# pc2/StencilStream

Hardware: NVIDIA B200
Metric: GCell-updates/s (higher is better)
Workload: dtype f32

## Files before the change

stencilstream_b200/include/StencilStream/cuda/internal/TileKernel.hpp:

```cpp
#pragma once
#include "../../Stencil.hpp"
#include "Helpers.hpp"

#include <cuda_runtime.h>

#include <cstddef>
#include <cstdint>
#include <type_traits>

namespace stencil {
namespace cuda {
namespace internal {

inline constexpr int store_tile = 0, store_grid = 1, store_runtime = 2;

template <typename Cell, int CW> constexpr bool lane_major_tiles() {
#if defined(STST_NO_LANE_MAJOR)
    return false;
#else
    using L = CellLayout<Cell>;
    if (!(CW == 4 || CW == 8))
        return false;
    const unsigned constant = constant_fields_mask<Cell>();
    unsigned evolving = 0;
    for (std::size_t i = 0; i < L::n_planes; i++) {
        if (L::plane_bytes(i) != 4)
            return false;
        if (!((constant >> i) & 1u))
            evolving++;
    }
  #if defined(STST_MIXED_LANE_MAJOR)
    return evolving == 1;
  #else
    return L::n_planes == 1 && evolving == 1;
  #endif
#endif
}

template <typename Cell, std::size_t I> constexpr bool plane_is_lane_major() {
    return ((constant_fields_mask<Cell>() >> I) & 1u) == 0;
}

inline constexpr int window_shift = 0, window_rotate = 1, window_reload = 2;

inline constexpr unsigned max_fused_iterations = 16;

inline constexpr unsigned max_spec_subiterations = 4;

struct SweepGeometry {
    unsigned grid_h, grid_w;
    int buf_row0;
    unsigned buf_rows;
    int out_row_lo;
    int out_row_hi;
    int out2_row_lo;
    int out2_row_hi;
    unsigned tiles_first;
    unsigned tile_h, tile_w;
    unsigned halo;
    unsigned hpad;
    unsigned n_gens;
    unsigned tiles_x;
    unsigned use_tma;
    unsigned push;
    unsigned inv_block_y;
    unsigned keep[max_spec_subiterations];
    unsigned probe;
    unsigned *spec_flags;
    unsigned long long iteration0;
};

template <typename TDV> struct TdvArray {
    TDV v[max_fused_iterations];
};

struct alignas(64) TensorMapSet {
    unsigned char map[max_planes][128];
};

struct HaloPush {
    PlaneSet up, down;
    int up_buf_row0, down_buf_row0;
    int up_row_hi;
    int down_row_lo;
    unsigned *ticket;
    unsigned *flag_up;
    unsigned *flag_down;
    unsigned flag_value;
};


template <typename T, int N> struct alignas((sizeof(T) * N) % 16 == 0 ? 16
                                            : (sizeof(T) * N) % 8 == 0 ? 8
                                            : (sizeof(T) * N) % 4 == 0 ? 4
                                                                       : alignof(T)) Pack {
    T v[N];
};

template <typename T>
inline constexpr bool is_shuffleable_v = std::is_trivially_copyable_v<T> &&
                                         (sizeof(T) == 1 || sizeof(T) == 2 || sizeof(T) == 4 ||
                                          sizeof(T) == 8);


inline constexpr unsigned tile_guard_bytes = 128;

template <typename Cell>
STST_HD inline std::size_t tile_buffer_bytes(unsigned tile_rows, unsigned tile_cols,
                                             unsigned without_planes = 0) {
    using L = CellLayout<Cell>;
    std::size_t total = 0;
    for (std::size_t i = 0; i < L::n_planes; i++) {
        if ((without_planes >> i) & 1u)
            continue;
        std::size_t b = std::size_t(tile_rows) * tile_cols * L::plane_bytes(i);
        total += (b + 127) / 128 * 128;
    }
    return total;
}

template <typename Cell>
STST_HD inline std::size_t tile_smem_bytes(unsigned tile_rows, unsigned tile_cols,
                                           unsigned n_buffers, unsigned single_planes = 0) {
    return tile_buffer_bytes<Cell>(tile_rows, tile_cols) +
           tile_buffer_bytes<Cell>(tile_rows, tile_cols, single_planes) * (n_buffers - 1) +
           2 * tile_guard_bytes;
}

#if defined(__CUDACC__)

template <typename To, typename From> __device__ __forceinline__ To bit_cast_dev(From const &f) {
    static_assert(sizeof(To) >= sizeof(From));
    To t{};
    memcpy(&t, &f, sizeof(From));
    return t;
}

template <typename T> __device__ __forceinline__ T from_bits(unsigned long long bits) {
    T t;
    memcpy(&t, &bits, sizeof(T));
    return t;
}

template <typename T> __device__ __forceinline__ T shuffle_from_lower_lane(T const &v) {
    if constexpr (sizeof(T) <= 4) {
        unsigned bits = bit_cast_dev<unsigned>(v);
        bits = __shfl_up_sync(0xffffffffu, bits, 1);
        return from_bits<T>(bits);
    } else {
        unsigned long long bits = bit_cast_dev<unsigned long long>(v);
        bits = __shfl_up_sync(0xffffffffu, bits, 1);
        return from_bits<T>(bits);
    }
}

template <typename T> __device__ __forceinline__ T shuffle_from_upper_lane(T const &v) {
    if constexpr (sizeof(T) <= 4) {
        unsigned bits = bit_cast_dev<unsigned>(v);
        bits = __shfl_down_sync(0xffffffffu, bits, 1);
        return from_bits<T>(bits);
    } else {
        unsigned long long bits = bit_cast_dev<unsigned long long>(v);
        bits = __shfl_down_sync(0xffffffffu, bits, 1);
        return from_bits<T>(bits);
    }
}

template <int Bytes>
__device__ __forceinline__ void cp_async_group(void *smem_dst, const void *gmem_src) {
    unsigned saddr = static_cast<unsigned>(__cvta_generic_to_shared(smem_dst));
    if constexpr (Bytes % 16 == 0) {
#pragma unroll
        for (int o = 0; o < Bytes; o += 16) {
            asm volatile("cp.async.cg.shared.global [%0], [%1], 16;\n" ::"r"(saddr + o),
                         "l"(static_cast<const char *>(gmem_src) + o)
                         : "memory");
        }
    } else if constexpr (Bytes == 8) {
        asm volatile("cp.async.ca.shared.global [%0], [%1], 8;\n" ::"r"(saddr), "l"(gmem_src)
                     : "memory");
    } else {
        static_assert(Bytes == 4);
        asm volatile("cp.async.ca.shared.global [%0], [%1], 4;\n" ::"r"(saddr), "l"(gmem_src)
                     : "memory");
    }
}

__device__ __forceinline__ void cp_async_wait_all() {
    asm volatile("cp.async.wait_all;\n" ::: "memory");
}


__device__ __forceinline__ void mbarrier_init(unsigned long long *bar, unsigned count) {
    unsigned addr = static_cast<unsigned>(__cvta_generic_to_shared(bar));
    asm volatile("mbarrier.init.shared::cta.b64 [%0], %1;\n" ::"r"(addr), "r"(count) : "memory");
}

__device__ __forceinline__ void fence_mbarrier_init() {
    asm volatile("fence.mbarrier_init.release.cluster;\n" ::: "memory");
}

__device__ __forceinline__ void fence_proxy_async() {
    asm volatile("fence.proxy.async.shared::cta;\n" ::: "memory");
}

__device__ __forceinline__ void mbarrier_arrive_expect_tx(unsigned long long *bar, unsigned bytes) {
    unsigned addr = static_cast<unsigned>(__cvta_generic_to_shared(bar));
    asm volatile("mbarrier.arrive.expect_tx.shared::cta.b64 _, [%0], %1;\n" ::"r"(addr), "r"(bytes)
                 : "memory");
}

__device__ __forceinline__ void mbarrier_wait_parity(unsigned long long *bar, unsigned parity) {
    unsigned addr = static_cast<unsigned>(__cvta_generic_to_shared(bar));
    unsigned done = 0;
    do {
        asm volatile("{\n"
                     ".reg .pred p;\n"
                     "mbarrier.try_wait.parity.shared::cta.b64 p, [%1], %2;\n"
                     "selp.u32 %0, 1, 0, p;\n"
                     "}\n"
                     : "=r"(done)
                     : "r"(addr), "r"(parity)
                     : "memory");
    } while (!done);
}

__device__ __forceinline__ void tma_load_2d(void *smem_dst, const void *tensor_map, int x, int y,
                                            unsigned long long *bar) {
    unsigned dst = static_cast<unsigned>(__cvta_generic_to_shared(smem_dst));
    unsigned mbar = static_cast<unsigned>(__cvta_generic_to_shared(bar));
    asm volatile("cp.async.bulk.tensor.2d.shared::cluster.global.mbarrier::complete_tx::bytes"
                 " [%0], [%1, {%3, %4}], [%2];\n" ::"r"(dst),
                 "l"(tensor_map), "r"(mbar), "r"(x), "r"(y)
                 : "memory");
}


template <typename Cell> struct TileView {
    using L = CellLayout<Cell>;
    unsigned char *base;
    unsigned rows, cols;
    unsigned plane_off[L::n_planes];

    __device__ __forceinline__ TileView(unsigned char *base, unsigned rows, unsigned cols)
        : base(base), rows(rows), cols(cols) {
        unsigned off = 0;
#pragma unroll
        for (unsigned i = 0; i < L::n_planes; i++) {
            plane_off[i] = off;
            unsigned b = rows * cols * unsigned(L::plane_bytes(i));
            off += (b + 127u) / 128u * 128u;
        }
    }

    __device__ __forceinline__ TileView(unsigned char *base, unsigned rows, unsigned cols, int)
        : base(base), rows(rows), cols(cols) {}

    template <std::size_t I> __device__ __forceinline__ typename L::template plane_t<I> *plane() const {
        return reinterpret_cast<typename L::template plane_t<I> *>(base + plane_off[I]);
    }
};


template <typename Cell, int CW, bool kInterior>
__device__ __forceinline__ void stage_tile(TileView<Cell> const &tile, PlaneSet const &src,
                                           TensorMapSet const &maps, SweepGeometry const &geo,
                                           Cell const &halo_value, int gy0, int gx0,
                                           unsigned long long *mbar) {
    using L = CellLayout<Cell>;
    const int c0 = int(threadIdx.x) * CW;
    const int gx = gx0 + c0;

    if (geo.use_tma) {
        if (threadIdx.x == 0 && threadIdx.y == 0) {
            unsigned total = 0;
            for_each_plane<Cell>([&](auto I) {
                total += tile.rows * tile.cols * unsigned(sizeof(typename L::template plane_t<I>));
            });
            mbarrier_arrive_expect_tx(mbar, total);
            for_each_plane<Cell>([&](auto I) {
                tma_load_2d(tile.template plane<I>(), &maps.map[I][0], gx0, gy0 - geo.buf_row0,
                            mbar);
            });
        }
        mbarrier_wait_parity(mbar, 0);
        if constexpr (!kInterior) {
            for (int row = int(threadIdx.y); row < int(tile.rows); row += int(blockDim.y)) {
                const int gy = gy0 + row;
                const bool row_in = gy >= 0 && gy < int(geo.grid_h);
                for_each_plane<Cell>([&](auto I) {
                    auto *s = tile.template plane<I>() + std::size_t(row) * tile.cols + c0;
#pragma unroll
                    for (int i = 0; i < CW; i++) {
                        const bool in = row_in && (gx + i) >= 0 && (gx + i) < int(geo.grid_w);
                        if (!in)
                            s[i] = L::template get<I>(halo_value);
                    }
                });
            }
            __syncthreads();
        }
        return;
    }

    for_each_plane<Cell>([&](auto I) {
        using T = typename L::template plane_t<I>;
        T *sp = tile.template plane<I>();
        const T *gp = static_cast<const T *>(src.base[I]);
        const unsigned long long pitch = src.pitch[I];
        for (int row = int(threadIdx.y); row < int(tile.rows); row += int(blockDim.y)) {
            const int gy = gy0 + row;
            T *s = sp + std::size_t(row) * tile.cols + c0;
            const T *g = gp + (long long)(gy - geo.buf_row0) * (long long)pitch + gx;
            if constexpr (kInterior) {
                if constexpr ((sizeof(T) * CW) % 16 == 0 || sizeof(T) * CW == 8 ||
                              sizeof(T) * CW == 4) {
                    cp_async_group<int(sizeof(T)) * CW>(s, g);
                } else {
                    *reinterpret_cast<Pack<T, CW> *>(s) = *reinterpret_cast<const Pack<T, CW> *>(g);
                }
            } else {
                const bool row_in = gy >= 0 && gy < int(geo.grid_h) &&
                                    unsigned(gy - geo.buf_row0) < geo.buf_rows;
                if (row_in && gx >= 0 && gx + CW <= int(geo.grid_w)) {
                    *reinterpret_cast<Pack<T, CW> *>(s) = *reinterpret_cast<const Pack<T, CW> *>(g);
                } else {
#pragma unroll
                    for (int i = 0; i < CW; i++) {
                        const bool in = row_in && (gx + i) >= 0 && (gx + i) < int(geo.grid_w);
                        s[i] = in ? g[i] : L::template get<I>(halo_value);
                    }
                }
            }
        }
    });
    if constexpr (kInterior)
        cp_async_wait_all();
    __syncthreads();
}


struct SpecTrack {
    unsigned keep;
    unsigned probe;
    unsigned changed;
    unsigned violated;
};

template <typename T> __device__ __forceinline__ bool bits_differ(T const &a, T const &b) {
    if constexpr (sizeof(T) == 1 || sizeof(T) == 2 || sizeof(T) == 4) {
        return bit_cast_dev<unsigned>(a) != bit_cast_dev<unsigned>(b);
    } else if constexpr (sizeof(T) == 8) {
        return bit_cast_dev<unsigned long long>(a) != bit_cast_dev<unsigned long long>(b);
    } else {
        const unsigned char *pa = reinterpret_cast<const unsigned char *>(&a);
        const unsigned char *pb = reinterpret_cast<const unsigned char *>(&b);
        bool d = false;
#pragma unroll
        for (unsigned i = 0; i < sizeof(T); i++)
            d |= pa[i] != pb[i];
        return d;
    }
}

template <typename F, int CW, bool kInterior, int kMode, int kStore, bool kInLaneMajor,
          bool kOutLaneMajor, int kTX, bool kSpec, std::size_t SUB>
__device__ __forceinline__ void
sweep_rows(F const &tf, typename F::Cell const &halo_value,
           typename F::TimeDependentValue const &tdv, std::size_t iteration,
           TileView<typename F::Cell> const &in, TileView<typename F::Cell> const &out,
           bool to_global_arg, PlaneSet const &dst, HaloPush const &push, SweepGeometry const &geo,
           int gy0, int gx0, int row_lo, int row_hi, int out_lo, int out_hi, SpecTrack &spec) {
    using Cell = typename F::Cell;
    using TDV = typename F::TimeDependentValue;
    using L = CellLayout<Cell>;
    using StencilImpl = Stencil<Cell, F::stencil_radius, TDV>;
    constexpr int R = int(F::stencil_radius);
    constexpr int D = 2 * R + 1;
    constexpr int WC = CW + 2 * R;
    static_assert(std::size_t(R) * L::max_plane_bytes() <= tile_guard_bytes,
                  "stencil radius times the widest field exceeds the shared-memory guard");

    const int cols = int(in.cols);
    const int c0 = int(threadIdx.x) * CW;
    const int lane = int(threadIdx.x) & 31;
    const int tx = int(threadIdx.x), TX = kTX ? kTX : int(blockDim.x);
    const bool to_global = kStore == store_runtime ? to_global_arg : (kStore == store_grid);

    const unsigned n_rows = unsigned(row_hi - row_lo);
    const int y_begin =
        row_lo + int((std::uint64_t(n_rows * threadIdx.y) * geo.inv_block_y) >> 24);
    const int y_end =
        row_lo + int((std::uint64_t(n_rows * (threadIdx.y + 1u)) * geo.inv_block_y) >> 24);
    if (y_begin >= y_end)
        return;

#if defined(STST_RELOAD_ROWS)
    constexpr int RPS = (kMode == window_reload) ? STST_RELOAD_ROWS : 1;
#else
    constexpr int RPS = 1;
#endif
    constexpr int DW = D + RPS - 1;
    Cell win[DW][WC];

    auto load_row = [&](Cell(&w)[WC], int row) {
        for_each_plane<Cell>([&](auto I) {
            using T = typename L::template plane_t<I>;
            const T *rp = in.template plane<I>() + row * cols;
            if constexpr (kInLaneMajor && plane_is_lane_major<Cell, I>()) {
                const T *q = rp + tx;
#pragma unroll
                for (int i = 0; i < CW; i++)
                    L::template get<I>(w[R + i]) = q[i * TX];
#pragma unroll
                for (int j = 1; j <= R; j++) {
                    L::template get<I>(w[R - j]) =
                        q[((CW - j % CW) % CW) * TX - (j + CW - 1) / CW];
                    L::template get<I>(w[R + CW - 1 + j]) = q[((j - 1) % CW) * TX + (j - 1) / CW + 1];
                }
                return;
            }
            const Pack<T, CW> p = *reinterpret_cast<const Pack<T, CW> *>(rp + c0);
#pragma unroll
            for (int i = 0; i < CW; i++)
                L::template get<I>(w[R + i]) = p.v[i];
#pragma unroll
            for (int j = 1; j <= R; j++) {
                T left, right;
#if defined(STST_EDGE_SHUFFLES)
                constexpr bool use_shuffles = true;
#else
                constexpr bool use_shuffles = false;
#endif
                if constexpr (is_shuffleable_v<T> && kMode != window_reload && use_shuffles) {
                    static_assert(R <= CW || sizeof(T) == 0,
                                  "edge shuffles reach one lane to each side only");
                    left = shuffle_from_lower_lane(p.v[CW - j]);
                    right = shuffle_from_upper_lane(p.v[j - 1]);
                    if (lane == 0)
                        left = rp[c0 - j];
                    if (lane == 31)
                        right = rp[c0 + CW - 1 + j];
                } else {
                    left = rp[c0 - j];
                    right = rp[c0 + CW - 1 + j];
                }
                L::template get<I>(w[R - j]) = left;
                L::template get<I>(w[R + CW - 1 + j]) = right;
            }
        });
    };

    auto compute_row = [&](auto top_c, int y) {
        constexpr int top = decltype(top_c)::value;
        const int gy = gy0 + y;
        Cell result[CW];
#pragma unroll
        for (int i = 0; i < CW; i++) {
            const int gx = gx0 + c0 + i;
            bool in_grid = true;
            if constexpr (!kInterior) {
                in_grid = gy >= 0 && gy < int(geo.grid_h) && gx >= 0 && gx < int(geo.grid_w);
            }
            if (in_grid) {
                const std::size_t id_r = std::size_t(unsigned(gy)), id_c = std::size_t(unsigned(gx));
                const std::size_t range_r = geo.grid_h, range_c = geo.grid_w;
                if constexpr (kInterior) {
                    __builtin_assume(id_r != 0);
                    __builtin_assume(id_r != range_r - 1);
                    __builtin_assume(id_r < range_r - 1);
                    __builtin_assume(id_r + 1 < range_r);
                    __builtin_assume(id_c != 0);
                    __builtin_assume(id_c != range_c - 1);
                    __builtin_assume(id_c < range_c - 1);
                    __builtin_assume(id_c + 1 < range_c);
                }
                StencilImpl st(sycl::id<2>(id_r, id_c), sycl::range<2>(range_r, range_c), iteration,
                               SUB, tdv);
#pragma unroll
                for (int sr = 0; sr < D; sr++) {
#pragma unroll
                    for (int sc = 0; sc < D; sc++) {
                        st[sycl::id<2>(sr, sc)] = win[(top + sr) % DW][i + sc];
                    }
                }
                result[i] = tf(st);
            } else {
                result[i] = halo_value;
            }
        }

        if constexpr (kSpec) {
            for_each_plane<Cell>([&](auto I) {
                const bool kept = (spec.keep >> I) & 1u;
                if (kept || spec.probe) {
                    bool differs = false;
#pragma unroll
                    for (int i = 0; i < CW; i++) {
                        bool in_grid = true;
                        if constexpr (!kInterior) {
                            const int gx = gx0 + c0 + i;
                            in_grid = gy >= 0 && gy < int(geo.grid_h) && gx >= 0 && gx < int(geo.grid_w);
                        }
                        if (in_grid)
                            differs |= bits_differ(L::template get<I>(result[i]),
                                                   L::template get<I>(win[(top + R) % DW][R + i]));
                    }
                    if (differs) {
                        spec.changed |= 1u << I;
                        if (kept)
                            spec.violated |= 1u << I;
                    }
                }
            });
        }

        if (!to_global) {
            for_each_plane<Cell>([&](auto I) {
                using T = typename L::template plane_t<I>;
                if constexpr (kSpec) {
                    if ((spec.keep >> I) & 1u)
                        return;
                }
                if constexpr (kOutLaneMajor && plane_is_lane_major<Cell, I>()) {
                    T *o = out.template plane<I>() + y * cols + tx;
#pragma unroll
                    for (int i = 0; i < CW; i++)
                        o[i * TX] = L::template get<I>(result[i]);
                } else {
                    Pack<T, CW> q;
#pragma unroll
                    for (int i = 0; i < CW; i++)
                        q.v[i] = L::template get<I>(result[i]);
                    *reinterpret_cast<Pack<T, CW> *>(out.template plane<I>() + y * cols + c0) = q;
                }
            });
        } else {
            const bool own_group = c0 >= int(geo.hpad) && c0 < int(geo.hpad + geo.tile_w);
            if (!own_group)
                return;
            const int gxg = gx0 + c0;
            if constexpr (!kInterior) {
                if (gy < out_lo || gy >= out_hi || gy >= int(geo.grid_h))
                    return;
            }
            auto store_row = [&](PlaneSet const &planes, int buf_row0) {
                for_each_plane<Cell>([&](auto I) {
                    using T = typename L::template plane_t<I>;
                    T *g = static_cast<T *>(planes.base[I]) +
                           (long long)(gy - buf_row0) * (long long)planes.pitch[I] + gxg;
                    if (kInterior || gxg + CW <= int(geo.grid_w)) {
                        Pack<T, CW> q;
#pragma unroll
                        for (int i = 0; i < CW; i++)
                            q.v[i] = L::template get<I>(result[i]);
                        *reinterpret_cast<Pack<T, CW> *>(g) = q;
                    } else {
#pragma unroll
                        for (int i = 0; i < CW; i++) {
                            if (gxg + i < int(geo.grid_w))
                                g[i] = L::template get<I>(result[i]);
                        }
                    }
                });
            };
            store_row(dst, geo.buf_row0);
            if (geo.push) {
                if (gy < push.up_row_hi)
                    store_row(push.up, push.up_buf_row0);
                if (gy >= push.down_row_lo)
                    store_row(push.down, push.down_buf_row0);
            }
        }
    };

    if constexpr (kMode != window_reload) {
#pragma unroll
        for (int j = 0; j < D - 1; j++)
            load_row(win[j], y_begin - R + j);
    }

    if constexpr (kMode == window_reload) {
        int y = y_begin;
        if constexpr (RPS > 1) {
            for (; y + RPS <= y_end; y += RPS) {
#pragma unroll
                for (int j = 0; j < DW; j++)
                    load_row(win[j], y - R + j);
                [&]<int... Us>(std::integer_sequence<int, Us...>) {
                    (compute_row(std::integral_constant<int, Us>{}, y + Us), ...);
                }(std::make_integer_sequence<int, RPS>{});
            }
        }
        for (; y < y_end; y++) {
#pragma unroll
            for (int j = 0; j < D; j++)
                load_row(win[j], y - R + j);
            compute_row(std::integral_constant<int, 0>{}, y);
        }
    } else if constexpr (kMode == window_rotate) {
        int y = y_begin;
        for (; y + D <= y_end; y += D) {
            [&]<int... Us>(std::integer_sequence<int, Us...>) {
                (
                    [&] {
                        load_row(win[(Us + D - 1) % D], y + Us + R);
                        compute_row(std::integral_constant<int, Us>{}, y + Us);
                    }(),
                    ...);
            }(std::make_integer_sequence<int, D>{});
        }
        if (y < y_end) {
            [&]<int... Us>(std::integer_sequence<int, Us...>) {
                (
                    [&] {
                        if (y + Us < y_end) {
                            load_row(win[(Us + D - 1) % D], y + Us + R);
                            compute_row(std::integral_constant<int, Us>{}, y + Us);
                        }
                    }(),
                    ...);
            }(std::make_integer_sequence<int, D>{});
        }
    } else {
        for (int y = y_begin; y < y_end; y++) {
            load_row(win[D - 1], y + R);
            compute_row(std::integral_constant<int, 0>{}, y);
#pragma unroll
            for (int j = 0; j < D - 1; j++) {
#pragma unroll
                for (int i = 0; i < WC; i++)
                    win[j][i] = win[j + 1][i];
            }
        }
    }
}


template <typename F, int CW, bool kInterior, int kMode, int kTX, bool kSpec>
__device__ __forceinline__ void
run_tile(F const &tf, typename F::Cell const &halo_value,
         TdvArray<typename F::TimeDependentValue> const &tdvs, PlaneSet const &src,
         PlaneSet const &dst, HaloPush const &push, TensorMapSet const &maps,
         SweepGeometry const &geo, unsigned char *smem, unsigned long long *mbar, int gy0,
         int gx0, int out_lo, int out_hi) {
    using Cell = typename F::Cell;
    using L = CellLayout<Cell>;
    constexpr int R = int(F::stencil_radius);
    constexpr unsigned n_sub = unsigned(F::n_subiterations);
    constexpr unsigned all_planes = (L::n_planes >= 32) ? ~0u : ((1u << L::n_planes) - 1u);

    const unsigned rows = geo.tile_h + 2 * geo.halo;
    const unsigned cols = blockDim.x * CW;
    const unsigned buffer_bytes = unsigned(tile_buffer_bytes<Cell>(rows, cols));

    TileView<Cell> buf0(smem + tile_guard_bytes, rows, cols);
    TileView<Cell> buf1(smem + tile_guard_bytes + buffer_bytes, rows, cols);

    unsigned single = 0, where = 0;
    unsigned changed[n_sub] = {};
    unsigned violated = 0;
    if constexpr (kSpec) {
        static_assert(n_sub <= max_spec_subiterations);
        single = all_planes;
#pragma unroll
        for (unsigned q = 0; q < n_sub; q++)
            single &= geo.keep[q];
        unsigned off = 0;
        for_each_plane<Cell>([&](auto I) {
            if ((single >> I) & 1u) {
                buf1.plane_off[I] = buf0.plane_off[I] - buffer_bytes;
            } else {
                buf1.plane_off[I] = off;
                off += (rows * cols * unsigned(L::plane_bytes(I)) + 127u) / 128u * 128u;
            }
        });
    }

    stage_tile<Cell, CW, kInterior>(buf0, src, maps, geo, halo_value, gy0, gx0, mbar);

    unsigned step = 0;
    for (unsigned g = 0; g < geo.n_gens; g++) {
        const std::size_t iteration = std::size_t(geo.iteration0) + g;
        const typename F::TimeDependentValue tdv = tdvs.v[g];
        [&]<std::size_t... Subs>(std::index_sequence<Subs...>) {
            (
                [&] {
                    const bool last = (g + 1 == geo.n_gens) && (Subs + 1 == n_sub);
                    const int lo = int(step + 1) * R;
                    const int hi = int(rows) - int(step + 1) * R;
                    constexpr bool kLM = lane_major_tiles<Cell, CW>() && kMode != window_reload;
                    constexpr std::size_t kSub = Subs;
                    SpecTrack track{0u, 0u, 0u, 0u};
                    auto run = [&](TileView<Cell> const &in, TileView<Cell> const &out) {
                        auto sweep = [&](auto store_c, auto in_lm_c, auto out_lm_c) {
                            sweep_rows<F, CW, kInterior, kMode, decltype(store_c)::value,
                                       decltype(in_lm_c)::value, decltype(out_lm_c)::value, kTX, kSpec,
                                       kSub>(tf, halo_value, tdv, iteration, in, out, last, dst, push,
                                             geo, gy0, gx0, lo, hi, out_lo, out_hi, track);
                        };
                        using std::false_type;
                        using std::true_type;
                        using grid_c = std::integral_constant<int, store_grid>;
                        using tile_c = std::integral_constant<int, store_tile>;
                        using runtime_c = std::integral_constant<int, store_runtime>;
                        if constexpr (kLM) {
                            if (step == 0) {
                                if (last)
                                    sweep(grid_c{}, false_type{}, false_type{});
                                else
                                    sweep(tile_c{}, false_type{}, true_type{});
                            } else {
                                if (last)
                                    sweep(grid_c{}, true_type{}, false_type{});
                                else
                                    sweep(tile_c{}, true_type{}, true_type{});
                            }
                        } else if constexpr (sizeof(Cell) <= 16) {
                            if (last)
                                sweep(grid_c{}, false_type{}, false_type{});
                            else
                                sweep(tile_c{}, false_type{}, false_type{});
                        } else {
                            sweep(runtime_c{}, false_type{}, false_type{});
                        }
                    };
                    if constexpr (kSpec) {
                        track.keep = geo.keep[kSub] & all_planes;
                        track.probe = geo.probe;
                        TileView<Cell> in(smem + tile_guard_bytes, rows, cols, 0);
                        TileView<Cell> out(smem + tile_guard_bytes, rows, cols, 0);
                        for_each_plane<Cell>([&](auto I) {
                            const unsigned a = buf0.plane_off[I];
                            const unsigned b = buffer_bytes + buf1.plane_off[I];
                            const bool in_second = (where >> I) & 1u;
                            in.plane_off[I] = in_second ? b : a;
                            out.plane_off[I] = ((track.keep >> I) & 1u) ? in.plane_off[I]
                                                                         : (in_second ? a : b);
                        });
                        run(in, out);
                        where ^= ~track.keep & all_planes;
                        changed[kSub] |= track.changed;
                        violated |= track.violated;
                    } else {
                        run((step & 1u) ? buf1 : buf0, (step & 1u) ? buf0 : buf1);
                    }
                    if (!last)
                        __syncthreads();
                    step++;
                }(),
                ...);
        }(std::make_index_sequence<n_sub>{});
    }

    if constexpr (kSpec) {
        violated = __reduce_or_sync(0xffffffffu, violated);
        const bool leader = (threadIdx.x & 31u) == 0;
        if (violated != 0 && leader)
            atomicOr(geo.spec_flags + max_spec_subiterations, violated);
        if (geo.probe) {
#pragma unroll
            for (unsigned q = 0; q < n_sub; q++) {
                const unsigned c = __reduce_or_sync(0xffffffffu, changed[q]);
                if (c != 0 && leader)
                    atomicOr(geo.spec_flags + q, c);
            }
        }
    }
}

template <typename F, int CW, int kMode, int kTX, int kMaxThreads, int kMinBlocks, bool kSpec = false>
__global__ void __launch_bounds__(kMaxThreads, kMinBlocks)
    fused_sweep_kernel(const __grid_constant__ F tf,
                       const __grid_constant__ typename F::Cell halo_value,
                       const __grid_constant__ TdvArray<typename F::TimeDependentValue> tdvs,
                       const __grid_constant__ PlaneSet src, const __grid_constant__ PlaneSet dst,
                       const __grid_constant__ HaloPush push,
                       const __grid_constant__ TensorMapSet maps,
                       const __grid_constant__ SweepGeometry geo) {
    extern __shared__ __align__(128) unsigned char smem[];
    __shared__ unsigned long long mbar;

    if (geo.use_tma) {
        if (threadIdx.x == 0 && threadIdx.y == 0) {
            mbarrier_init(&mbar, 1);
            fence_mbarrier_init();
        }
        __syncthreads();
    }

    unsigned tile_index = blockIdx.x;
    int out_lo = geo.out_row_lo, out_hi = geo.out_row_hi;
    if (tile_index >= geo.tiles_first) {
        tile_index -= geo.tiles_first;
        out_lo = geo.out2_row_lo;
        out_hi = geo.out2_row_hi;
    }
    const unsigned tx = tile_index % geo.tiles_x;
    const unsigned ty = tile_index / geo.tiles_x;
    const int tile_gy = out_lo + int(ty * geo.tile_h);
    const int tile_gx = int(tx * geo.tile_w);
    const int gy0 = tile_gy - int(geo.halo);
    const int gx0 = tile_gx - int(geo.hpad);

    const bool interior = gy0 >= 0 && tile_gy + int(geo.tile_h + geo.halo) <= int(geo.grid_h) &&
                          tile_gy + int(geo.tile_h) <= out_hi && gx0 >= 1 &&
                          tile_gx + int(geo.tile_w + geo.hpad) + 1 <= int(geo.grid_w);

    if (interior) {
        run_tile<F, CW, true, kMode, kTX, kSpec>(tf, halo_value, tdvs, src, dst, push, maps, geo, smem,
                                                 &mbar, gy0, gx0, out_lo, out_hi);
    } else {
        run_tile<F, CW, false, (kMode == window_reload ? window_reload : window_shift), kTX, kSpec>(
            tf, halo_value, tdvs, src, dst, push, maps, geo, smem, &mbar, gy0, gx0, out_lo, out_hi);
    }

    if (geo.push && push.ticket != nullptr && blockIdx.x < gridDim.x) {
        __threadfence_system();
        __syncthreads();
        if (threadIdx.x == 0 && threadIdx.y == 0) {
            const unsigned ticket = atomicAdd(push.ticket, 1u);
            if (ticket == gridDim.x - 1u) {
                __threadfence_system();
                if (push.flag_up != nullptr)
                    *reinterpret_cast<volatile unsigned *>(push.flag_up) = push.flag_value;
                if (push.flag_down != nullptr)
                    *reinterpret_cast<volatile unsigned *>(push.flag_down) = push.flag_value;
                *reinterpret_cast<volatile unsigned *>(push.ticket) = 0u;
                __threadfence_system();
            }
        }
    }
}


template <typename Cell>
__global__ void __launch_bounds__(256)
    scatter_cells_kernel(const Cell *__restrict__ aos, PlaneSet planes, unsigned long long width,
                         unsigned long long plane_row0, unsigned long long n_cells) {
    using L = CellLayout<Cell>;
    const unsigned long long stride = (unsigned long long)gridDim.x * blockDim.x;
    for (unsigned long long idx = (unsigned long long)blockIdx.x * blockDim.x + threadIdx.x;
         idx < n_cells; idx += stride) {
        const unsigned long long r = idx / width, c = idx - r * width;
        const Cell cell = aos[idx];
        for_each_plane<Cell>([&](auto I) {
            using T = typename L::template plane_t<I>;
            static_cast<T *>(planes.base[I])[(plane_row0 + r) * planes.pitch[I] + c] =
                L::template get<I>(cell);
        });
    }
}

template <typename Cell>
__global__ void __launch_bounds__(256)
    gather_cells_kernel(Cell *__restrict__ aos, PlaneSet planes, unsigned long long width,
                        unsigned long long plane_row0, unsigned long long n_cells) {
    using L = CellLayout<Cell>;
    const unsigned long long stride = (unsigned long long)gridDim.x * blockDim.x;
    for (unsigned long long idx = (unsigned long long)blockIdx.x * blockDim.x + threadIdx.x;
         idx < n_cells; idx += stride) {
        const unsigned long long r = idx / width, c = idx - r * width;
        Cell cell;
        for_each_plane<Cell>([&](auto I) {
            using T = typename L::template plane_t<I>;
            L::template get<I>(cell) =
                static_cast<const T *>(planes.base[I])[(plane_row0 + r) * planes.pitch[I] + c];
        });
        aos[idx] = cell;
    }
}

#endif

}
}
}
```

Before: 1727.

## Fuse pairs of generations into one register-resident sweep for radius-1 stencils

```diff
diff --git a/stencilstream_b200/include/StencilStream/cuda/internal/TileKernel.hpp b/stencilstream_b200/include/StencilStream/cuda/internal/TileKernel.hpp
--- a/stencilstream_b200/include/StencilStream/cuda/internal/TileKernel.hpp
+++ b/stencilstream_b200/include/StencilStream/cuda/internal/TileKernel.hpp
@@ -42,6 +42,15 @@
 }
 
 inline constexpr int window_shift = 0, window_rotate = 1, window_reload = 2;
+
+template <typename F, int CW, int kMode, bool kSpec> constexpr bool paired_sweeps() {
+#if defined(STST_SINGLE_SWEEPS)
+    return false;
+#else
+    return lane_major_tiles<typename F::Cell, CW>() && CellLayout<typename F::Cell>::n_planes == 1 &&
+           F::stencil_radius == 1 && F::n_subiterations == 1 && kMode == window_rotate && !kSpec;
+#endif
+}
 
 inline constexpr unsigned max_fused_iterations = 16;
 
@@ -363,6 +372,91 @@
     }
 }
 
+__device__ __forceinline__ void row_group_rows(SweepGeometry const &geo, int row_lo, int row_hi,
+                                               int &y_begin, int &y_end) {
+    const unsigned n_rows = unsigned(row_hi - row_lo);
+    y_begin = row_lo + int((std::uint64_t(n_rows * threadIdx.y) * geo.inv_block_y) >> 24);
+    y_end = row_lo + int((std::uint64_t(n_rows * (threadIdx.y + 1u)) * geo.inv_block_y) >> 24);
+}
+
+__device__ __forceinline__ void assume_inside_grid(std::size_t id_r, std::size_t id_c,
+                                                   std::size_t range_r, std::size_t range_c) {
+    __builtin_assume(id_r != 0);
+    __builtin_assume(id_r != range_r - 1);
+    __builtin_assume(id_r < range_r - 1);
+    __builtin_assume(id_r + 1 < range_r);
+    __builtin_assume(id_c != 0);
+    __builtin_assume(id_c != range_c - 1);
+    __builtin_assume(id_c < range_c - 1);
+    __builtin_assume(id_c + 1 < range_c);
+}
+
+template <typename Cell, int CW, bool kInterior, bool kOutLaneMajor, int kTX>
+__device__ __forceinline__ void
+store_cells(Cell const (&result)[CW], int y, int gy, bool to_global, unsigned keep,
+            TileView<Cell> const &out, PlaneSet const &dst, HaloPush const &push,
+            SweepGeometry const &geo, int gx0, int out_lo, int out_hi) {
+    using L = CellLayout<Cell>;
+    const int cols = int(out.cols);
+    const int c0 = int(threadIdx.x) * CW;
+    const int tx = int(threadIdx.x), TX = kTX ? kTX : int(blockDim.x);
+    if (!to_global) {
+        for_each_plane<Cell>([&](auto I) {
+            using T = typename L::template plane_t<I>;
+            if ((keep >> I) & 1u)
+                return;
+            if constexpr (kOutLaneMajor && plane_is_lane_major<Cell, I>()) {
+                T *o = out.template plane<I>() + y * cols + tx;
+#pragma unroll
+                for (int i = 0; i < CW; i++)
+                    o[i * TX] = L::template get<I>(result[i]);
+            } else {
+                Pack<T, CW> q;
+#pragma unroll
+                for (int i = 0; i < CW; i++)
+                    q.v[i] = L::template get<I>(result[i]);
+                *reinterpret_cast<Pack<T, CW> *>(out.template plane<I>() + y * cols + c0) = q;
+            }
+        });
+    } else {
+        const bool own_group = c0 >= int(geo.hpad) && c0 < int(geo.hpad + geo.tile_w);
+        if (!own_group)
+            return;
+        const int gxg = gx0 + c0;
+        if constexpr (!kInterior) {
+            if (gy < out_lo || gy >= out_hi || gy >= int(geo.grid_h))
+                return;
+        }
+        auto store_row = [&](PlaneSet const &planes, int buf_row0) {
+            for_each_plane<Cell>([&](auto I) {
+                using T = typename L::template plane_t<I>;
+                T *g = static_cast<T *>(planes.base[I]) +
+                       (long long)(gy - buf_row0) * (long long)planes.pitch[I] + gxg;
+                if (kInterior || gxg + CW <= int(geo.grid_w)) {
+                    Pack<T, CW> q;
+#pragma unroll
+                    for (int i = 0; i < CW; i++)
+                        q.v[i] = L::template get<I>(result[i]);
+                    *reinterpret_cast<Pack<T, CW> *>(g) = q;
+                } else {
+#pragma unroll
+                    for (int i = 0; i < CW; i++) {
+                        if (gxg + i < int(geo.grid_w))
+                            g[i] = L::template get<I>(result[i]);
+                    }
+                }
+            });
+        };
+        store_row(dst, geo.buf_row0);
+        if (geo.push) {
+            if (gy < push.up_row_hi)
+                store_row(push.up, push.up_buf_row0);
+            if (gy >= push.down_row_lo)
+                store_row(push.down, push.down_buf_row0);
+        }
+    }
+}
+
 template <typename F, int CW, bool kInterior, int kMode, int kStore, bool kInLaneMajor,
           bool kOutLaneMajor, int kTX, bool kSpec, std::size_t SUB>
 __device__ __forceinline__ void
@@ -387,11 +481,8 @@
     const int tx = int(threadIdx.x), TX = kTX ? kTX : int(blockDim.x);
     const bool to_global = kStore == store_runtime ? to_global_arg : (kStore == store_grid);
 
-    const unsigned n_rows = unsigned(row_hi - row_lo);
-    const int y_begin =
-        row_lo + int((std::uint64_t(n_rows * threadIdx.y) * geo.inv_block_y) >> 24);
-    const int y_end =
-        row_lo + int((std::uint64_t(n_rows * (threadIdx.y + 1u)) * geo.inv_block_y) >> 24);
+    int y_begin, y_end;
+    row_group_rows(geo, row_lo, row_hi, y_begin, y_end);
     if (y_begin >= y_end)
         return;
 
@@ -465,16 +556,8 @@
             if (in_grid) {
                 const std::size_t id_r = std::size_t(unsigned(gy)), id_c = std::size_t(unsigned(gx));
                 const std::size_t range_r = geo.grid_h, range_c = geo.grid_w;
-                if constexpr (kInterior) {
-                    __builtin_assume(id_r != 0);
-                    __builtin_assume(id_r != range_r - 1);
-                    __builtin_assume(id_r < range_r - 1);
-                    __builtin_assume(id_r + 1 < range_r);
-                    __builtin_assume(id_c != 0);
-                    __builtin_assume(id_c != range_c - 1);
-                    __builtin_assume(id_c < range_c - 1);
-                    __builtin_assume(id_c + 1 < range_c);
-                }
+                if constexpr (kInterior)
+                    assume_inside_grid(id_r, id_c, range_r, range_c);
                 StencilImpl st(sycl::id<2>(id_r, id_c), sycl::range<2>(range_r, range_c), iteration,
                                SUB, tdv);
 #pragma unroll
@@ -515,63 +598,9 @@
             });
         }
 
-        if (!to_global) {
-            for_each_plane<Cell>([&](auto I) {
-                using T = typename L::template plane_t<I>;
-                if constexpr (kSpec) {
-                    if ((spec.keep >> I) & 1u)
-                        return;
-                }
-                if constexpr (kOutLaneMajor && plane_is_lane_major<Cell, I>()) {
-                    T *o = out.template plane<I>() + y * cols + tx;
-#pragma unroll
-                    for (int i = 0; i < CW; i++)
-                        o[i * TX] = L::template get<I>(result[i]);
-                } else {
-                    Pack<T, CW> q;
-#pragma unroll
-                    for (int i = 0; i < CW; i++)
-                        q.v[i] = L::template get<I>(result[i]);
-                    *reinterpret_cast<Pack<T, CW> *>(out.template plane<I>() + y * cols + c0) = q;
-                }
-            });
-        } else {
-            const bool own_group = c0 >= int(geo.hpad) && c0 < int(geo.hpad + geo.tile_w);
-            if (!own_group)
-                return;
-            const int gxg = gx0 + c0;
-            if constexpr (!kInterior) {
-                if (gy < out_lo || gy >= out_hi || gy >= int(geo.grid_h))
-                    return;
-            }
-            auto store_row = [&](PlaneSet const &planes, int buf_row0) {
-                for_each_plane<Cell>([&](auto I) {
-                    using T = typename L::template plane_t<I>;
-                    T *g = static_cast<T *>(planes.base[I]) +
-                           (long long)(gy - buf_row0) * (long long)planes.pitch[I] + gxg;
-                    if (kInterior || gxg + CW <= int(geo.grid_w)) {
-                        Pack<T, CW> q;
-#pragma unroll
-                        for (int i = 0; i < CW; i++)
-                            q.v[i] = L::template get<I>(result[i]);
-                        *reinterpret_cast<Pack<T, CW> *>(g) = q;
-                    } else {
-#pragma unroll
-                        for (int i = 0; i < CW; i++) {
-                            if (gxg + i < int(geo.grid_w))
-                                g[i] = L::template get<I>(result[i]);
-                        }
-                    }
-                });
-            };
-            store_row(dst, geo.buf_row0);
-            if (geo.push) {
-                if (gy < push.up_row_hi)
-                    store_row(push.up, push.up_buf_row0);
-                if (gy >= push.down_row_lo)
-                    store_row(push.down, push.down_buf_row0);
-            }
-        }
+        store_cells<Cell, CW, kInterior, kOutLaneMajor, kTX>(result, y, gy, to_global,
+                                                             kSpec ? spec.keep : 0u, out, dst, push,
+                                                             geo, gx0, out_lo, out_hi);
     };
 
     if constexpr (kMode != window_reload) {
@@ -633,6 +662,133 @@
                     win[j][i] = win[j + 1][i];
             }
         }
+    }
+}
+
+template <int V> using int_c = std::integral_constant<int, V>;
+
+template <typename F, int CW, int kStore, bool kInLaneMajor, int kTX>
+__device__ __forceinline__ void
+sweep_pair(F const &tf, typename F::TimeDependentValue const &tdv1,
+           typename F::TimeDependentValue const &tdv2, std::size_t iteration,
+           TileView<typename F::Cell> const &in, TileView<typename F::Cell> const &out,
+           PlaneSet const &dst, HaloPush const &push, SweepGeometry const &geo, int gy0, int gx0,
+           int row_lo, int row_hi, int out_lo, int out_hi) {
+    using Cell = typename F::Cell;
+    using TDV = typename F::TimeDependentValue;
+    using L = CellLayout<Cell>;
+    using T = typename L::template plane_t<0>;
+    using StencilImpl = Stencil<Cell, 1, TDV>;
+    static_assert(L::n_planes == 1 && F::stencil_radius == 1 && CW % 2 == 0);
+    constexpr int W0 = CW + 4, W1 = CW + 2;
+
+    const int cols = int(in.cols);
+    const int c0 = int(threadIdx.x) * CW;
+    const int tx = int(threadIdx.x), TX = kTX ? kTX : int(blockDim.x);
+
+    int y_begin, y_end;
+    row_group_rows(geo, row_lo, row_hi, y_begin, y_end);
+    if (y_begin >= y_end)
+        return;
+
+    Cell w0[3][W0];
+    Cell w1[3][W1];
+
+    auto load_row = [&](auto slot_c, int row) {
+        Cell(&w)[W0] = w0[decltype(slot_c)::value];
+        const T *rp = in.template plane<0>() + row * cols;
+        if constexpr (kInLaneMajor) {
+            const T *q = rp + tx;
+#pragma unroll
+            for (int i = 0; i < CW; i++)
+                L::template get<0>(w[2 + i]) = q[i * TX];
+            L::template get<0>(w[0]) = q[(CW - 2) * TX - 1];
+            L::template get<0>(w[1]) = q[(CW - 1) * TX - 1];
+            L::template get<0>(w[CW + 2]) = q[1];
+            L::template get<0>(w[CW + 3]) = q[TX + 1];
+        } else {
+            const Pack<T, CW> p = *reinterpret_cast<const Pack<T, CW> *>(rp + c0);
+            const Pack<T, 2> l = *reinterpret_cast<const Pack<T, 2> *>(rp + c0 - 2);
+            const Pack<T, 2> r = *reinterpret_cast<const Pack<T, 2> *>(rp + c0 + CW);
+#pragma unroll
+            for (int i = 0; i < CW; i++)
+                L::template get<0>(w[2 + i]) = p.v[i];
+            L::template get<0>(w[0]) = l.v[0];
+            L::template get<0>(w[1]) = l.v[1];
+            L::template get<0>(w[CW + 2]) = r.v[0];
+            L::template get<0>(w[CW + 3]) = r.v[1];
+        }
+    };
+
+    auto apply = [&](auto inside_c, auto const &nb, int gy, int gx, std::size_t it,
+                     TDV const &tdv) -> Cell {
+        const std::size_t id_r = std::size_t(unsigned(gy)), id_c = std::size_t(unsigned(gx));
+        const std::size_t range_r = geo.grid_h, range_c = geo.grid_w;
+        if constexpr (decltype(inside_c)::value)
+            assume_inside_grid(id_r, id_c, range_r, range_c);
+        StencilImpl st(sycl::id<2>(id_r, id_c), sycl::range<2>(range_r, range_c), it, 0, tdv);
+#pragma unroll
+        for (int sr = 0; sr < 3; sr++) {
+#pragma unroll
+            for (int sc = 0; sc < 3; sc++)
+                st[sycl::id<2>(sr, sc)] = nb(sr, sc);
+        }
+        return tf(st);
+    };
+
+    auto first = [&](auto top_c, auto slot_c, int y) {
+        constexpr int top = decltype(top_c)::value;
+#pragma unroll
+        for (int i = 0; i < W1; i++) {
+            auto nb = [&](int sr, int sc) -> Cell const & { return w0[(top + sr) % 3][i + sc]; };
+            const int gx = gx0 + c0 - 1 + i;
+            if (i == 0 || i == W1 - 1)
+                w1[decltype(slot_c)::value][i] =
+                    apply(std::false_type{}, nb, gy0 + y, gx, iteration, tdv1);
+            else
+                w1[decltype(slot_c)::value][i] =
+                    apply(std::true_type{}, nb, gy0 + y, gx, iteration, tdv1);
+        }
+    };
+
+    auto second = [&](auto top_c, int y) {
+        constexpr int top = decltype(top_c)::value;
+        const int gy = gy0 + y;
+        Cell result[CW];
+#pragma unroll
+        for (int i = 0; i < CW; i++) {
+            auto nb = [&](int sr, int sc) -> Cell const & { return w1[(top + sr) % 3][i + sc]; };
+            result[i] = apply(std::true_type{}, nb, gy, gx0 + c0 + i, iteration + 1, tdv2);
+        }
+        store_cells<Cell, CW, true, kStore == store_tile, kTX>(result, y, gy, kStore == store_grid, 0u,
+                                                               out, dst, push, geo, gx0, out_lo,
+                                                               out_hi);
+    };
+
+    auto row_step = [&](auto u_c, int y) {
+        constexpr int u = decltype(u_c)::value;
+        load_row(int_c<(u + 1) % 3>{}, y + 2);
+        first(int_c<(u + 2) % 3>{}, int_c<(u + 2) % 3>{}, y + 1);
+        second(int_c<u>{}, y);
+    };
+
+    load_row(int_c<0>{}, y_begin - 2);
+    load_row(int_c<1>{}, y_begin - 1);
+    load_row(int_c<2>{}, y_begin);
+    first(int_c<0>{}, int_c<0>{}, y_begin - 1);
+    load_row(int_c<0>{}, y_begin + 1);
+    first(int_c<1>{}, int_c<1>{}, y_begin);
+
+    int y = y_begin;
+    for (; y + 3 <= y_end; y += 3) {
+        row_step(int_c<0>{}, y);
+        row_step(int_c<1>{}, y + 1);
+        row_step(int_c<2>{}, y + 2);
+    }
+    if (y < y_end) {
+        row_step(int_c<0>{}, y);
+        if (y + 1 < y_end)
+            row_step(int_c<1>{}, y + 1);
     }
 }
 
@@ -678,6 +834,55 @@
     }
 
     stage_tile<Cell, CW, kInterior>(buf0, src, maps, geo, halo_value, gy0, gx0, mbar);
+
+    if constexpr (kInterior && paired_sweeps<F, CW, kMode, kSpec>()) {
+        using grid_c = std::integral_constant<int, store_grid>;
+        using tile_c = std::integral_constant<int, store_tile>;
+        unsigned g = 0;
+        bool flip = false;
+        if (geo.n_gens & 1u) {
+            const bool last = geo.n_gens == 1;
+            SpecTrack track{0u, 0u, 0u, 0u};
+            auto sweep = [&](auto store_c, auto out_lm_c) {
+                sweep_rows<F, CW, true, kMode, decltype(store_c)::value, false,
+                           decltype(out_lm_c)::value, kTX, false, 0>(
+                    tf, halo_value, tdvs.v[0], std::size_t(geo.iteration0), buf0, buf1, last, dst,
+                    push, geo, gy0, gx0, R, int(rows) - R, out_lo, out_hi, track);
+            };
+            if (last) {
+                sweep(grid_c{}, std::false_type{});
+                return;
+            }
+            sweep(tile_c{}, std::true_type{});
+            __syncthreads();
+            g = 1;
+            flip = true;
+        }
+        for (; g < geo.n_gens; g += 2) {
+            const bool last = g + 2 == geo.n_gens;
+            auto pair = [&](auto store_c, auto in_lm_c) {
+                sweep_pair<F, CW, decltype(store_c)::value, decltype(in_lm_c)::value, kTX>(
+                    tf, tdvs.v[g], tdvs.v[g + 1], std::size_t(geo.iteration0) + g,
+                    flip ? buf1 : buf0, flip ? buf0 : buf1, dst, push, geo, gy0, gx0,
+                    int(g + 2) * R, int(rows) - int(g + 2) * R, out_lo, out_hi);
+            };
+            if (g == 0) {
+                if (last)
+                    pair(grid_c{}, std::false_type{});
+                else
+                    pair(tile_c{}, std::false_type{});
+            } else {
+                if (last)
+                    pair(grid_c{}, std::true_type{});
+                else
+                    pair(tile_c{}, std::true_type{});
+            }
+            if (!last)
+                __syncthreads();
+            flip = !flip;
+        }
+        return;
+    }
 
     unsigned step = 0;
     for (unsigned g = 0; g < geo.n_gens; g++) {
```

Result: faster. 2025 (median of 6 runs) (+17.3%).
